# adolliou/euispice_coreg

Measured on AMD Instinct MI355X. Metric: lag-points/sec (whole node) on 2048² grid, 60×60 CRVAL sweep; argmax-shift match, higher is better.
Workload: dtype f64; 1 GPU; headline: Carrington 'fa' 2048x2048 grid lon(200,300) lat(-20,20), 60x60 CRVAL lags arange(-30,30,1) arcsec, small 2048^2 HRIEUV-like, ref 3072^2 FSI-like, order 2, solar_r 1.004; lag_points=3600, parallelism=single GPU, no collective, resident=True, sweeps_in_flight=2, small_stored_f32=True, use_lds=True

## Files before the change

### euispice_coreg_amd/csrc/coreg_hip.hip

```cpp
#include <hip/hip_runtime.h>

#include <algorithm>
#include <chrono>
#include <cmath>
#include <cstdio>
#include <cstdlib>
#include <cstring>
#include <limits>
#include <condition_variable>
#include <map>
#include <memory>
#include <mutex>
#include <string>
#include <thread>
#include <functional>
#include <type_traits>
#include <utility>
#include <vector>

#include "fit.hpp"
#include "geometry.hpp"
#include "kernels.hpp"
#include <atomic>
#include "ricecomp.hpp"
#include "riceenc.hpp"

using namespace coreg;

#define COREG_VERSION "0.1.0"

#include "lag_plan.hpp"
#include "sweep_plan.hpp"
#include "host_owned.hpp"
#include "host_state.hpp"
#include "host_upload.hpp"
#include "host_plan.hpp"
#include "host_fix_launch.hpp"
#include "sweep_variant.hpp"
#include "host_sweep_launch.hpp"
#include "host_sweep_mi.hpp"
#include "host_fix_lists.hpp"
#include "host_sweep_io.hpp"
#include "host_context.hpp"
#include "pixels_plan.hpp"
#include "host_pixels.hpp"

coreg_handle::~coreg_handle() = default;

extern "C" {

const char* coreg_version(void) { return "coreg_hip " COREG_VERSION " (gfx950)"; }

int coreg_create(coreg_handle** out, int device) {
    if (!out) return COREG_EINVAL;
    *out = nullptr;
    int ndev = 0;
    hipError_t e = hipGetDeviceCount(&ndev);
    if (e != hipSuccess || ndev < 1) return COREG_EHIP;
    if (device < 0) {
        if (hipGetDevice(&device) != hipSuccess) device = 0;
    }
    if (device >= ndev) return COREG_EINVAL;
    coreg_handle* h = new (std::nothrow) coreg_handle();
    if (!h) return COREG_ENOMEM;
    h->device = device;
    if (hipSetDevice(device) != hipSuccess || hipStreamCreateWithFlags(&h->stream.s, hipStreamNonBlocking) != hipSuccess ||
        hipEventCreate(&h->ev_end[0].e) != hipSuccess ||
        hipEventCreate(&h->ev_end[1].e) != hipSuccess || hipEventRecord(h->ev_end[0], h->stream) != hipSuccess ||
        hipEventRecord(h->ev_end[1], h->stream) != hipSuccess ||
        h->pivots.reserve(2 * sizeof(double)) != hipSuccess ||
        hipMemsetAsync(h->pivots.p, 0, 2 * sizeof(double), h->stream) != hipSuccess) {
        coreg_destroy(h);
        return COREG_EHIP;
    }
    std::memset(&h->stats, 0, sizeof(h->stats));
    *out = h;
    return COREG_OK;
}

void coreg_destroy(coreg_handle* h) {
    if (!h) return;
    (void)hipSetDevice(h->device);
    if (h->up_thread.joinable()) {
        {
            std::unique_lock<std::mutex> lk(h->up_m);
            h->up_cv.wait(lk, [&] { return !h->up_busy && !h->up_has; });
            h->up_stop = true;
        }
        h->up_cv.notify_all();
        h->up_thread.join();
    }
    if (h->stream) (void)hipStreamSynchronize(h->stream);
    if (h->up_stream) (void)hipStreamSynchronize(h->up_stream);
    delete h;
}

const char* coreg_last_error(const coreg_handle* h) { return h ? h->err.c_str() : "null handle"; }

int coreg_set_stream(coreg_handle* h, void* hip_stream) {
    if (!h) return COREG_EINVAL;
    RETCHK(bind_device(h));
    RETCHK(collect_stats(h));
    HIPCHK(hipStreamSynchronize(h->stream));
    HIPCHK(h->stream.borrow((hipStream_t)hip_stream));
    return COREG_OK;
}

int coreg_synchronize(coreg_handle* h) {
    if (!h) return COREG_EINVAL;
    RETCHK(bind_device(h));
    HIPCHK(hipStreamSynchronize(h->stream));
    return COREG_OK;
}

int coreg_set_option(coreg_handle* h, const char* name, int64_t value) {
    if (!h || !name) return COREG_EINVAL;
    const std::string n(name);
    if (n == "use_lds") {
        h->opt_use_lds = value ? 1 : 0;
    } else if (n == "clean_path") {
        h->opt_clean_path = value ? 1 : 0;
    } else if (n == "tap_nan_filter") {
        if (value < 0 || value > 2) return fail(h, COREG_EINVAL, "tap_nan_filter must be 0, 1 or 2");
        h->opt_tap_nan_filter = value;
    } else if (n == "overlap_upload") {
        h->opt_overlap_upload = value ? 1 : 0;
    } else if (n == "async_upload") {
        h->opt_async_upload = value ? 1 : 0;
    } else if (n == "refine") {
        h->opt_refine = value ? 1 : 0;
    } else if (n == "refine_cond_log10") {
        if (value < -3 || value > 15) return fail(h, COREG_EINVAL, "refine_cond_log10 must be in [-3, 15]");
        h->opt_refine_cond_log10 = value;
    } else if (n == "refine_max") {
        if (value < 0 || value > 16) return fail(h, COREG_EINVAL, "refine_max must be in [0, 16]");
    } else if (n == "tile_w") {
        if (value != 0 && (value < 1 || value > kTilePts || (value & (value - 1)) != 0))
            return fail(h, COREG_EINVAL, "tile_w must be 0 or a power of two <= 1024");
        h->opt_tile_w = value;
    } else if (n == "n_groups") {
        if (value < 0) return fail(h, COREG_EINVAL, "n_groups must be >= 0");
        h->opt_n_groups = value;
    } else if (n == "skew") {
        (void)value;
    } else if (n == "shard_world") {
        if (value < 1 || value > 64) return fail(h, COREG_EINVAL, "shard_world must be in [1, 64]");
        h->opt_shard_world = value;
        if (h->opt_shard_rank >= value) h->opt_shard_rank = 0;
    } else if (n == "combo_begin") {
        if (value < 0) return fail(h, COREG_EINVAL, "combo_begin must be >= 0");
        h->opt_combo_begin = value;
    } else if (n == "combo_end") {
        if (value < 0) return fail(h, COREG_EINVAL, "combo_end must be >= 0");
        h->opt_combo_end = value;
    } else if (n == "shard_rank") {
        if (value < 0 || value >= h->opt_shard_world) return fail(h, COREG_EINVAL, "shard_rank must be in [0, shard_world)");
        h->opt_shard_rank = value;
    } else if (n == "border_fix") {
        h->opt_border_fix = value ? 1 : 0;
    } else if (n == "tap_fix") {
        h->opt_tap_fix = value ? 1 : 0;
    } else if (n == "tap_cap") {
        if (value < 1 || value > (1 << 26)) return fail(h, COREG_EINVAL, "tap_cap must be in [1, 2^26]");
        h->opt_tap_cap = value;
    } else if (n == "pitch") {
        h->opt_pitch = value;
    } else if (n == "taper_frac") {
        if (value < -1 || value > 1000) return fail(h, COREG_EINVAL, "taper_frac must be in [-1, 1000]");
        h->opt_taper_frac = value;
    } else if (n == "taper_min") {
        if (value < 16 || value > 1024) return fail(h, COREG_EINVAL, "taper_min must be in [16, 1024]");
        h->opt_taper_min = value;
    } else if (n == "taper_rounds") {
        if (value < 1) return fail(h, COREG_EINVAL, "taper_rounds must be >= 1");
        h->opt_taper_rounds = value;
    } else if (n == "crop_reference") {
        h->opt_crop_reference = value ? 1 : 0;
    } else if (n == "tile_skip") {
        h->opt_tile_skip = value ? 1 : 0;
    } else if (n == "h_series") {
        h->opt_h_series = value ? 1 : 0;
    } else if (n == "h_incr") {
        h->opt_h_incr = value ? 1 : 0;
    } else if (n == "patch_w") {
        if (value < 0 || value > kBlock) return fail(h, COREG_EINVAL, "patch_w must be in [0, 256]");
        h->opt_patch_w = value;
    } else if (n == "mi_chunks") {
        if (value < 0 || value > kMiMaxChunks) return fail(h, COREG_EINVAL, "mi_chunks must be in [0, 64]");
        h->opt_mi_chunks = value;
    } else if (n == "lds_bytes") {
        if (value < 1024 || value > 159 * 1024) return fail(h, COREG_EINVAL, "lds_bytes must be in [1 KiB, 159 KiB]");
        h->opt_lds_bytes = value;
    } else {
        return fail(h, COREG_EINVAL, "unknown option: " + n);
    }
    return COREG_OK;
}

}

#include "abi_images.hpp"
#include "abi_sweeps.hpp"
#include "abi_host.hpp"
#include "abi_context.hpp"
#include "abi_pixels.hpp"


#include "multi.hpp"
```

### euispice_coreg_amd/csrc/host_state.hpp

```cpp
#pragma once
namespace {

enum SrcKind {
    SRC_HOST = 0,
    SRC_PINNED = 1,
    SRC_DEVICE = 2,
    SRC_TILED = 3,
};

struct PixFmt {
    int bitpix = 0;
    bool f32 = false;
    double bscale = 1.0, bzero = 0.0;
    bool raw() const { return bitpix != 0; }
    bool scaled() const { return bscale != 1.0 || bzero != 0.0; }
    size_t elem() const { return raw() ? (size_t)(bitpix < 0 ? -bitpix : bitpix) / 8 : (f32 ? 4 : 8); }
    bool swap_only() const { return bitpix == -32 && !scaled(); }
    static PixFmt native(bool is_f32) {
        PixFmt f;
        f.f32 = is_f32;
        return f;
    }
};

constexpr int kMaxDevices = 64;
std::mutex g_attr_mutex;

struct EventPair {
    Event a, b;
    bool b_is_next_sweep = false;
    size_t next_sweep_index = 0;
};

}

struct KeptTapLists {
    DevBuf all;
};
struct TapFix {
    TapFixArgs args = {};
    int segs = 0;
    int mode = 0;
    long long count = 0;
};
struct FixLaunch {
    std::vector<BorderFixArgs> border;
    std::vector<ParityFixArgs> parity;
    TapFix tap;
    std::shared_ptr<KeptTapLists> kept;
    bool small_f32 = true;
    bool empty() const { return border.empty() && parity.empty() && tap.segs == 0; }
};

struct ContextState;
struct PixelsState;

struct coreg_handle {
    int device = 0;
    Stream stream;
    std::string err;

    std::unique_ptr<ContextState> ctx;
    std::unique_ptr<PixelsState> pix;
    ~coreg_handle();

    DevBuf small;
    int sW = 0, sH = 0;
    bool small_f32 = false;
    DevBuf ref;
    int gW = 0, gH = 0;
    int ref_dtype = -1;
    DevBuf pivots, red_sum, red_cnt;
    DevBuf t_sin_lon, t_cos_lon, t_cos_lat, t_sin_lat, t_lon_deg, t_dx;
    coreg_diffrot rot_ref = {}, rot_small = {};
    bool has_rot_ref = false, has_rot_small = false;
    CarrTables tabs;
    std::vector<double> tabs_key;
    bool tabs_uploaded = false;
    PinBuf pin_img[2];
    Event ev_img[2];
    int pin_img_next = 0;
    DevBuf pts, tile_count, tile_list, tile_cum, group_first, tile_info, tile_bbox;
    DevBuf visit_rec;
    DevBuf rf_fix_slab;
    DevBuf counters;
    DevBuf lane_params, out_index, partials, out_dev, tmp_img;
    DevBuf counts;
    long long counts_n = -1;
    DevBuf up_f64, up_flag;
    DevBuf up_raw;
    DevBuf rice_blob, rice_rand, dec_img;
    PrologueArgs pending_prologue = {};
    DevBuf bbox_buf;
    Stream aux_stream;
    Stream up_stream;
    Event ev_small, ev_main;
    bool small_pending = false;
    DevBuf red_sum_up, red_cnt_up;
    int64_t opt_overlap_upload = 1;
    int64_t opt_tap_nan_filter = 2;
    int64_t opt_async_upload = 0;
    std::thread up_thread;
    std::mutex up_m;
    std::condition_variable up_cv;
    std::function<hipError_t()> up_job;
    bool up_has = false, up_stop = false, up_busy = false;
    hipError_t up_rc = hipSuccess;
    PinBuf pin_small[2];
    Event ev_pin_small[2];
    int pin_small_next = 0;
    WcslibCaches wcslib;
    DevBuf border_flags, fix_partial;
    DevBuf border_dev;
    PinBuf pin_border;
    int64_t opt_border_fix = 1;
    int64_t opt_tap_fix = 1, opt_tap_cap = 1 << 24;
    DevBuf tap_count, tap_segq, tap_list, tap_skip, tap_seg_slot, tap_seg_begin, tap_pixel, tap_xw, tap_yw;
    long long tap_last[3] = {0, 0, 0};
    int last_variant[7] = {-1, 0, 0, 0, 0, 0, 0};
    int64_t opt_shard_world = 1, opt_shard_rank = 0;
    int64_t opt_combo_begin = 0, opt_combo_end = 0;
    DevBuf sums;
    long long sums_slots = 0;
    struct PendingFinalize {
        long long slot_off, n_slots, lag_begin;
        int residus;
        RefineArgs refine;
        std::function<int(coreg_handle*)> replay_precompute;
        FixLaunch fixes;
    };
    std::function<int(coreg_handle*)> last_precompute;
    PlanMemo plan_memo;
    DevBuf rf_flags, rf_pivots, rf_list, rf_head, rf_partial;
    std::vector<PendingFinalize> pending_fin;
    DevBuf fin_outidx;
    long long pending_n_out = 0;
    std::vector<double> mi_edges_small, mi_edges_large;
    DevBuf mi_hist;
    size_t mi_lds[6] = {0, 0, 0, 0, 0, 0};
    int64_t opt_mi_chunks = 0;

    int64_t opt_crop_reference = 1;
    int64_t opt_taper_min = 128, opt_taper_frac = -1, opt_taper_rounds = 6;
    int64_t opt_use_lds = 1, opt_clean_path = 1, opt_refine = 1, opt_refine_cond_log10 = 5, opt_tile_w = 0, opt_n_groups = 0, opt_lds_bytes = (159 * 1024 * kPointGroups) / 4, opt_patch_w = 0, opt_h_series = 1, opt_h_incr = 1, opt_tile_skip = 1, opt_pitch = -1;

    coreg_stats stats;
    bool stats_pending = false;
    PinBuf pin_info;
    std::vector<EventPair> ev_sweep, ev_pre;
    size_t ev_sweep_used = 0, ev_pre_used = 0;
    hipEvent_t ev_t1 = nullptr;
    Event ev_end[2];
    PinBuf pin_plan[2];
    int plan_slot = 0;
    bool plan_open = false;
};
```

### euispice_coreg_amd/csrc/host_sweep_launch.hpp

```cpp
#pragma once
namespace {
using sweep_variant::SweepVariant;
static_assert(sweep_variant::kTranslate == MODE_TRANSLATE && sweep_variant::kHomography == MODE_HOMOGRAPHY &&
                  sweep_variant::kHomographySeries == MODE_HOMOGRAPHY_SERIES && sweep_variant::kCar == MODE_CAR &&
                  sweep_variant::kOrderRt == ORDER_RT, "sweep_variant.hpp restates the kernels' constants");

struct SweepLaunchSpec {
    int mode = MODE_TRANSLATE;
    int order = 2;
    int method = COREG_METHOD_CORRELATION;
    size_t slot_off = 0;
    int n_batches = 0, n_tiles = 0;
    long long lag_begin = 0;
    double* out_dev = nullptr;
    const LaunchU* car_inv = nullptr;
    const BorderFix* fix = nullptr;
    int pitch_sel = 0;
    long long n_slots() const { return (long long)n_batches * kBlock; }
    bool residus() const { return method != COREG_METHOD_CORRELATION; }
    int residus_kind() const { return method == COREG_METHOD_RESIDUS_MASKED ? 2 : (residus() ? 1 : 0); }
    const double* params_dev(const coreg_handle* h) const {
        return h->lane_params.as<double>() + (mode == MODE_TRANSLATE ? 2 : 9) * slot_off;
    }
    const long long* outidx_dev(const coreg_handle* h) const { return h->out_index.as<long long>() + slot_off; }
};

struct SweepKernel {
    void (*fn)(const SweepArgs);
    size_t attr_bytes[kMaxDevices];
};
template <size_t... I>
SweepKernel* sweep_kernel_table(std::index_sequence<I...>) {
    constexpr const SweepVariant* v = sweep_variant::kSweepVariants.v;
    static SweepKernel table[] = {
        {k_sweep<v[I].mode, v[I].order, std::conditional_t<v[I].f32, float, double>, v[I].round, v[I].resid, v[I].pitch>, {0}}...};
    return table;
}

int raise_dynamic_lds(coreg_handle* h, SweepKernel* k, size_t lds_bytes) {
    std::lock_guard<std::mutex> lock(g_attr_mutex);
    size_t& ab = k->attr_bytes[h->device % kMaxDevices];
    if (lds_bytes > 48 * 1024 && lds_bytes > ab) {
        HIPCHK(hipFuncSetAttribute((const void*)k->fn, hipFuncAttributeMaxDynamicSharedMemorySize, (int)lds_bytes));
        ab = lds_bytes;
    }
    return COREG_OK;
}

int launch_k_sweep(coreg_handle* h, const SweepLaunchSpec& L, const SweepArgs& a, dim3 grid, size_t lds_bytes) {
    const SweepVariant v = sweep_variant::pick_sweep_variant(L.mode, L.order, h->small_f32, L.residus(), L.pitch_sel);
    const int at = sweep_variant::sweep_variant_index(v);
    if (at < 0) return fail(h, COREG_EINVAL, "launch_sweep: no k_sweep instantiation for this mode / order / pitch");
    SweepKernel* k = sweep_kernel_table(std::make_index_sequence<sweep_variant::kNumSweepVariants>()) + at;
    EventPair* ev = next_event(h, h->ev_sweep, h->ev_sweep_used);
    if (!ev) return fail(h, COREG_EHIP, "hipEventCreate failed");
    RETCHK(raise_dynamic_lds(h, k, lds_bytes));
    HIPCHK(hipEventRecord(ev->a, h->stream));
    hipLaunchKernelGGL(k->fn, grid, dim3(kSweepThreads), lds_bytes, h->stream, a);
    HIPCHK(hipEventRecord(ev->b, h->stream));
    HIPCHK(hipGetLastError());
    const int rec[7] = {at, v.mode, v.order, v.f32 ? 1 : 0, v.round ? 1 : 0, v.resid ? 1 : 0, v.pitch};
    std::copy(rec, rec + 7, h->last_variant);
    return COREG_OK;
}

SweepArgs sweep_args(const coreg_handle* h, const SweepLaunchSpec& L, int n_groups, int group_lo, size_t lds_bytes) {
    SweepArgs a;
    a.img = h->small.p;
    a.W = h->sW;
    a.H = h->sH;
    a.pts = h->pts.as<Pt>();
    a.tile_count = h->tile_count.as<int>();
    a.tile_list = h->tile_list.as<int>();
    a.tile_cum = h->tile_cum.as<int>();
    a.group_first = h->group_first.as<int>();
    a.tile_info = h->tile_info.as<long long>();
    a.tile_bbox = h->tile_bbox.as<double>();
    a.visit_rec = h->visit_rec.as<VisitRec>();
    a.lane_params = L.params_dev(h);
    a.n_slots = L.n_slots();
    a.n_batches = L.n_batches;
    a.n_groups = n_groups;
    a.group_lo = group_lo;
    a.partials = h->partials.as<double>();
    a.pivots = h->pivots.as<double>();
    a.use_lds = h->opt_use_lds ? 1 : 0;
    a.clean_path = h->opt_clean_path ? 1 : 0;
    a.lds_elems = (int)(lds_bytes / sizeof(double));
    a.car_inv = L.car_inv ? *L.car_inv : LaunchU{};
    a.car_inv.order_rt = L.order;
    a.car_inv.h_incr = (int)h->opt_h_incr;
    return a;
}

template <typename Args>
void fill_fix_common(Args& x, const coreg_handle* h, const SweepLaunchSpec& L) {
    x.img = h->small.p;
    x.W = h->sW;
    x.H = h->sH;
    x.ref = h->ref.p;
    x.ref_f32 = h->ref_dtype == COREG_F32 ? 1 : 0;
    x.gw = h->gW;
    x.order = L.order;
    x.round_f32 = L.mode == MODE_TRANSLATE ? 0 : 1;
    x.residus = L.residus() ? 1 : 0;
    x.pivots = h->pivots.as<double>();
    x.hom = L.params_dev(h);
    x.n_slots = L.n_slots();
}

int build_fix_launch(coreg_handle* h, const SweepLaunchSpec& L, FixLaunch* fl) {
    fl->small_f32 = h->small_f32;
    if (!L.fix || !L.fix->any()) return COREG_OK;
    static const std::vector<BorderItems::Item> no_items;
    for (const BorderItems::Item& it : L.fix->border ? L.fix->border->items : no_items) {
        if (it.flags_off >= 0) {
            ParityFixArgs p = {};
            fill_fix_common(p, h, L);
            p.flags = h->border_flags.as<unsigned char>() + it.flags_off;
            p.gh = h->gH;
            p.slot = it.slot;
            p.n_partial = 256;
            if (h->fix_partial.reserve((size_t)p.n_partial * kNumSums * sizeof(double)) != hipSuccess)
                return fail(h, COREG_EHIP, "hipMalloc failed (parity fix)");
            p.partial = h->fix_partial.as<double>();
            fl->parity.push_back(p);
        }
        if (it.n == 0) continue;
        BorderFixArgs b = {};
        fill_fix_common(b, h, L);
        b.slot = it.slot;
        b.dropped = h->border_dev.as<int>() + it.first;
        b.n_dropped = it.n;
        fl->border.push_back(b);
    }
    if (L.fix->tap.segs > 0) {
        fl->tap = L.fix->tap;
        fill_fix_common(fl->tap.args, h, L);
    }
    return COREG_OK;
}

int keep_tap_lists(coreg_handle* h, FixLaunch* fixes) {
    auto kept = std::make_shared<KeptTapLists>();
    const size_t nseg = (size_t)fixes->tap.segs, cnt = (size_t)fixes->tap.count;
    TapFixArgs& t = fixes->tap.args;
    const void* src[5] = {t.xw, t.yw, t.pixel, t.seg_begin, t.seg_slot};
    const size_t bytes[5] = {cnt * sizeof(double), cnt * sizeof(double), cnt * sizeof(unsigned), (nseg + 1) * sizeof(int),
                             nseg * sizeof(int)};
    size_t off[6] = {0};
    for (int k = 0; k < 5; ++k) off[k + 1] = off[k] + ((bytes[k] + 7) & ~(size_t)7);
    HIPCHK(kept->all.reserve(off[5]));
    char* all = kept->all.as<char>();
    for (int k = 0; k < 5; ++k)
        if (bytes[k]) HIPCHK(hipMemcpyAsync(all + off[k], src[k], bytes[k], hipMemcpyDeviceToDevice, h->stream));
    t.xw = (const double*)(all + off[0]);
    t.yw = (const double*)(all + off[1]);
    t.pixel = (const unsigned*)(all + off[2]);
    t.seg_begin = (const int*)(all + off[3]);
    t.seg_slot = (const int*)(all + off[4]);
    fixes->kept = kept;
    return COREG_OK;
}

int queue_pending_finalize(coreg_handle* h, const SweepLaunchSpec& L, const RefineArgs& refine, bool refinable,
                           const FixLaunch& fl) {
    coreg_handle::PendingFinalize pf;
    pf.slot_off = (long long)L.slot_off;
    pf.n_slots = L.n_slots();
    pf.lag_begin = L.lag_begin;
    pf.residus = L.residus_kind();
    pf.refine = refine;
    pf.refine.enabled = refinable ? 1 : 0;
    pf.replay_precompute = h->last_precompute;
    pf.fixes = fl;
    if (L.mode == MODE_CAR && fl.tap.segs > 0) RETCHK(keep_tap_lists(h, &pf.fixes));
    h->pending_fin.push_back(pf);
    return COREG_OK;
}

int launch_sweep(coreg_handle* h, const SweepLaunchSpec& L) {
    const long long n_slots = L.n_slots();
    const int n_groups = pick_groups(h, L.n_batches, L.n_tiles);
    const bool sharded = h->opt_shard_world > 1;
    const int g_per = sharded ? n_groups / (int)h->opt_shard_world : n_groups;
    const int g_lo = sharded ? g_per * (int)h->opt_shard_rank : 0;
    const bool fixing = L.fix && L.fix->any() && (!sharded || h->opt_shard_rank == 0);
    HIPCHK(h->partials.reserve((size_t)(g_per + (fixing ? 1 : 0)) * kNumSums * n_slots * sizeof(double)));
    double* fix_slab = fixing ? h->partials.as<double>() + (size_t)g_per * kNumSums * n_slots : nullptr;
    const size_t lds_min = (size_t)(kPointGroups - 1) * kNumSums * kBlock * sizeof(double);
    const size_t lds_bytes = std::max(lds_min, h->opt_use_lds ? (size_t)h->opt_lds_bytes : 0);

    const SweepArgs a = sweep_args(h, L, n_groups, g_lo, lds_bytes);
    RETCHK(join_small(h));
    trace("launch_sweep: launching k_sweep");
    RETCHK(launch_k_sweep(h, L, a, dim3((unsigned)((long long)g_per * L.n_batches)), lds_bytes));
    h->stats.n_sweep_launches++;
    h->stats.used_lds = a.use_lds;

    FixLaunch fl;
    RETCHK(build_fix_launch(h, L, &fl));
    if (fixing) {
        HIPCHK(hipMemsetAsync(fix_slab, 0, (size_t)kNumSums * n_slots * sizeof(double), h->stream));
        RETCHK(launch_fix_kernels(h, fl, fix_slab, nullptr, nullptr));
    }

    const bool refinable = h->opt_refine && !L.residus();
    FinalizeArgs f = {};
    RETCHK(fill_refine(h, &f.refine, L.mode, L.order, a.lane_params, a.car_inv, n_slots));
    f.refine.enabled = (refinable && !sharded) ? 1 : 0;
    if (fixing && f.refine.enabled) {
        HIPCHK(h->rf_fix_slab.reserve((size_t)kNumSums * n_slots * sizeof(double)));
        f.refine.fix_slab = h->rf_fix_slab.as<double>();
    }
    f.fix_slab = fix_slab;
    f.refine_count = h->counters.as<long long>();
    f.partials = h->partials.as<double>();
    f.n_groups = g_per + (fixing ? 1 : 0);
    f.part_stride = n_slots;
    if (sharded) {
        f.sums_out = h->sums.as<double>();
        f.sums_stride = h->sums_slots;
        f.sums_off = (long long)L.slot_off;
    }
    f.n_slots = n_slots;
    f.out_index = L.outidx_dev(h);
    f.lag_begin = L.lag_begin;
    f.out = L.out_dev;
    f.counts = h->counts.as<double>();
    f.residus = L.residus_kind();
    f.n_required = (long long)h->gW * h->gH;
    launch_finalize(h, f);
    HIPCHK(hipGetLastError());

    if (sharded) return queue_pending_finalize(h, L, f.refine, refinable, fl);
    if (!f.refine.enabled) return COREG_OK;
    hipLaunchKernelGGL(k_refine_list, dim3(1), dim3(kListThreads), 0, h->stream, f.refine, n_slots, h->counters.as<long long>());
    return refine_with_fixes(h, f.refine, fl, n_slots, f.out_index, L.lag_begin, L.out_dev);
}

}
```

### euispice_coreg_amd/csrc/kernels_sweep.hpp

```cpp
#pragma once
namespace coreg {
struct SweepArgs {
    const void* img;
    int W, H;
    const Pt* pts;
    const int* tile_count;
    const int* tile_list;
    const int* tile_cum;
    const int* group_first;
    long long* tile_info;
    const double* tile_bbox;
    const VisitRec* visit_rec;
    const double* lane_params;
    long long n_slots;
    int n_batches;
    int n_groups;
    int group_lo;
    double* partials;
    const double* pivots;
    int use_lds;
    int clean_path;
    int lds_elems;
    LaunchU car_inv;
};

struct Acc {
    int n;
    double a, b, aa, bb, ab;
};

template <int N>
struct Taps;
template <>
struct Taps<3> {
    double t[9];
    __device__ __forceinline__ void issue(unsigned a0, unsigned a1, unsigned a2) {
        asm volatile(
            "ds_read_b64 %0, %9\n\tds_read_b64 %1, %9 offset:8\n\tds_read_b64 %2, %9 offset:16\n\t"
            "ds_read_b64 %3, %10\n\tds_read_b64 %4, %10 offset:8\n\tds_read_b64 %5, %10 offset:16\n\t"
            "ds_read_b64 %6, %11\n\tds_read_b64 %7, %11 offset:8\n\tds_read_b64 %8, %11 offset:16"
            : "=&v"(t[0]), "=&v"(t[1]), "=&v"(t[2]), "=&v"(t[3]), "=&v"(t[4]), "=&v"(t[5]), "=&v"(t[6]), "=&v"(t[7]),
              "=&v"(t[8])
            : "v"(a0), "v"(a1), "v"(a2));
    }
    __device__ __forceinline__ void wait_after(double& w0, double& w1, double& w2, double& w3, double& w4, double& w5) {
        asm volatile("s_waitcnt lgkmcnt(0)"
                     : "+v"(t[0]), "+v"(t[1]), "+v"(t[2]), "+v"(t[3]), "+v"(t[4]), "+v"(t[5]), "+v"(t[6]), "+v"(t[7]),
                       "+v"(t[8]), "+v"(w0), "+v"(w1), "+v"(w2), "+v"(w3), "+v"(w4), "+v"(w5));
    }
    __device__ __forceinline__ void issue_before(unsigned a0, unsigned a1, unsigned a2, double& fx, double& fy) {
        asm volatile(
            "ds_read_b64 %0, %11\n\tds_read_b64 %1, %11 offset:8\n\tds_read_b64 %2, %11 offset:16\n\t"
            "ds_read_b64 %3, %12\n\tds_read_b64 %4, %12 offset:8\n\tds_read_b64 %5, %12 offset:16\n\t"
            "ds_read_b64 %6, %13\n\tds_read_b64 %7, %13 offset:8\n\tds_read_b64 %8, %13 offset:16"
            : "=&v"(t[0]), "=&v"(t[1]), "=&v"(t[2]), "=&v"(t[3]), "=&v"(t[4]), "=&v"(t[5]), "=&v"(t[6]), "=&v"(t[7]),
              "=&v"(t[8]), "+v"(fx), "+v"(fy)
            : "v"(a0), "v"(a1), "v"(a2));
    }
    __device__ __forceinline__ void wait() {
        asm volatile("s_waitcnt lgkmcnt(0)"
                     : "+v"(t[0]), "+v"(t[1]), "+v"(t[2]), "+v"(t[3]), "+v"(t[4]), "+v"(t[5]), "+v"(t[6]), "+v"(t[7]),
                       "+v"(t[8]));
    }
    template <int P>
    __device__ __forceinline__ void issue_before_imm(unsigned a0, double& fx, double& fy) {
        static_assert(P > 0 && (2 * P + 2) * 8 < 65536, "LDS immediate offsets are 16 bits");
        asm volatile(
            "ds_read_b64 %0, %11\n\tds_read_b64 %1, %11 offset:8\n\tds_read_b64 %2, %11 offset:16\n\t"
            "ds_read_b64 %3, %11 offset:%12\n\tds_read_b64 %4, %11 offset:%13\n\tds_read_b64 %5, %11 offset:%14\n\t"
            "ds_read_b64 %6, %11 offset:%15\n\tds_read_b64 %7, %11 offset:%16\n\tds_read_b64 %8, %11 offset:%17"
            : "=&v"(t[0]), "=&v"(t[1]), "=&v"(t[2]), "=&v"(t[3]), "=&v"(t[4]), "=&v"(t[5]), "=&v"(t[6]), "=&v"(t[7]),
              "=&v"(t[8]), "+v"(fx), "+v"(fy)
            : "v"(a0), "n"(P * 8), "n"(P * 8 + 8), "n"(P * 8 + 16), "n"(2 * P * 8), "n"(2 * P * 8 + 8),
              "n"(2 * P * 8 + 16));
    }
};
template <>
struct Taps<2> {
    double t[4];
    __device__ __forceinline__ void issue(unsigned a0, unsigned a1, unsigned) {
        asm volatile(
            "ds_read_b64 %0, %4\n\tds_read_b64 %1, %4 offset:8\n\t"
            "ds_read_b64 %2, %5\n\tds_read_b64 %3, %5 offset:8"
            : "=&v"(t[0]), "=&v"(t[1]), "=&v"(t[2]), "=&v"(t[3])
            : "v"(a0), "v"(a1));
    }
    __device__ __forceinline__ void issue_before(unsigned a0, unsigned a1, unsigned a2, double&, double&) {
        issue(a0, a1, a2);
    }
    __device__ __forceinline__ void wait_after(double&, double&, double&, double&, double&, double&) { wait(); }
    __device__ __forceinline__ void wait() {
        asm volatile("s_waitcnt lgkmcnt(0)" : "+v"(t[0]), "+v"(t[1]), "+v"(t[2]), "+v"(t[3]));
    }
};

template <>
struct Taps<4> {
    double t[16];
    __device__ __forceinline__ void issue_before(unsigned a0, unsigned a1, unsigned a2, unsigned a3, double& fx,
                                                 double& fy) {
        asm volatile(
            "ds_read_b64 %0, %18\n\tds_read_b64 %1, %18 offset:8\n\tds_read_b64 %2, %18 offset:16\n\t"
            "ds_read_b64 %3, %18 offset:24\n\t"
            "ds_read_b64 %4, %19\n\tds_read_b64 %5, %19 offset:8\n\tds_read_b64 %6, %19 offset:16\n\t"
            "ds_read_b64 %7, %19 offset:24\n\t"
            "ds_read_b64 %8, %20\n\tds_read_b64 %9, %20 offset:8\n\tds_read_b64 %10, %20 offset:16\n\t"
            "ds_read_b64 %11, %20 offset:24\n\t"
            "ds_read_b64 %12, %21\n\tds_read_b64 %13, %21 offset:8\n\tds_read_b64 %14, %21 offset:16\n\t"
            "ds_read_b64 %15, %21 offset:24"
            : "=&v"(t[0]), "=&v"(t[1]), "=&v"(t[2]), "=&v"(t[3]), "=&v"(t[4]), "=&v"(t[5]), "=&v"(t[6]), "=&v"(t[7]),
              "=&v"(t[8]), "=&v"(t[9]), "=&v"(t[10]), "=&v"(t[11]), "=&v"(t[12]), "=&v"(t[13]), "=&v"(t[14]),
              "=&v"(t[15]), "+v"(fx), "+v"(fy)
            : "v"(a0), "v"(a1), "v"(a2), "v"(a3));
    }
    template <int P>
    __device__ __forceinline__ void issue_before_imm(unsigned a0, double& fx, double& fy) {
        static_assert(P > 0 && (3 * P + 3) * 8 < 65536, "LDS immediate offsets are 16 bits");
        asm volatile(
            "ds_read_b64 %0, %18\n\tds_read_b64 %1, %18 offset:8\n\tds_read_b64 %2, %18 offset:16\n\t"
            "ds_read_b64 %3, %18 offset:24\n\t"
            "ds_read_b64 %4, %18 offset:%19\n\tds_read_b64 %5, %18 offset:%20\n\tds_read_b64 %6, %18 offset:%21\n\t"
            "ds_read_b64 %7, %18 offset:%22\n\t"
            "ds_read_b64 %8, %18 offset:%23\n\tds_read_b64 %9, %18 offset:%24\n\tds_read_b64 %10, %18 offset:%25\n\t"
            "ds_read_b64 %11, %18 offset:%26\n\t"
            "ds_read_b64 %12, %18 offset:%27\n\tds_read_b64 %13, %18 offset:%28\n\tds_read_b64 %14, %18 offset:%29\n\t"
            "ds_read_b64 %15, %18 offset:%30"
            : "=&v"(t[0]), "=&v"(t[1]), "=&v"(t[2]), "=&v"(t[3]), "=&v"(t[4]), "=&v"(t[5]), "=&v"(t[6]), "=&v"(t[7]),
              "=&v"(t[8]), "=&v"(t[9]), "=&v"(t[10]), "=&v"(t[11]), "=&v"(t[12]), "=&v"(t[13]), "=&v"(t[14]),
              "=&v"(t[15]), "+v"(fx), "+v"(fy)
            : "v"(a0), "n"(P * 8), "n"(P * 8 + 8), "n"(P * 8 + 16), "n"(P * 8 + 24), "n"(2 * P * 8), "n"(2 * P * 8 + 8),
              "n"(2 * P * 8 + 16), "n"(2 * P * 8 + 24), "n"(3 * P * 8), "n"(3 * P * 8 + 8), "n"(3 * P * 8 + 16),
              "n"(3 * P * 8 + 24));
    }
    __device__ __forceinline__ void wait_after(double* wx, double* wy) {
        asm volatile("s_waitcnt lgkmcnt(0)"
                     : "+v"(t[0]), "+v"(t[1]), "+v"(t[2]), "+v"(t[3]), "+v"(t[4]), "+v"(t[5]), "+v"(t[6]), "+v"(t[7]),
                       "+v"(t[8]), "+v"(t[9]), "+v"(t[10]), "+v"(t[11]), "+v"(t[12]), "+v"(t[13]), "+v"(t[14]),
                       "+v"(t[15]), "+v"(wx[0]), "+v"(wx[1]), "+v"(wx[2]), "+v"(wx[3]), "+v"(wy[0]), "+v"(wy[1]),
                       "+v"(wy[2]), "+v"(wy[3]));
    }
};

template <int PITCH, bool FOLDED = false>
__device__ __forceinline__ double gather_o3(unsigned win, int pitch, double cx, double cy, double offx, double offy) {
    int c0, r0;
    double fx, fy;
    if constexpr (FOLDED) {
        c0 = (int)cx;
        r0 = (int)cy;
        fx = __builtin_amdgcn_fract(cx);
        fy = __builtin_amdgcn_fract(cy);
    } else {
        const double flx = floor(cx), fly = floor(cy);
        c0 = (int)flx + (int)offx;
        r0 = (int)fly + (int)offy;
        fx = cx - flx;
        fy = cy - fly;
    }
    const unsigned a0 = win + 8u * (unsigned)(__mul24(r0, PITCH > 0 ? PITCH : pitch) + c0);
    Taps<4> tp;
    if constexpr (PITCH > 0) {
        tp.template issue_before_imm<PITCH>(a0, fx, fy);
    } else {
        const unsigned a1 = a0 + 8u * (unsigned)pitch;
        const unsigned a2 = a1 + 8u * (unsigned)pitch;
        const unsigned a3 = a2 + 8u * (unsigned)pitch;
        tp.issue_before(a0, a1, a2, a3, fx, fy);
    }
    double wx[4], wy[4];
    spline_weights6_o3(fx, wx);
    spline_weights6_o3(fy, wy);
// ... 328 lines not shown
        const unsigned lo = (unsigned)__builtin_amdgcn_readlane(w, 3 + 2 * k);
        const unsigned hi = (unsigned)__builtin_amdgcn_readlane(w, 4 + 2 * k);
        b[k] = __builtin_bit_cast(double, ((unsigned long long)hi << 32) | (unsigned long long)lo);
    }
    v.bx0 = b[0];
    v.bx1 = b[1];
    v.by0 = b[2];
    v.by1 = b[3];
}

template <int MODE, int ORDER, typename TS, bool LDS, bool ROUND, bool RESID, bool INTERIOR = false, int PITCH = 0,
          bool CLEAN = false>
__device__ __forceinline__ void tile_points(Acc& acc, unsigned win, const TS* __restrict__ img, int pitch,
                                            int ox, int oy, int W, int H, double px0, double py0, double pxw,
                                            double pyw, const H9& hm, const LaunchU& cu, const Pt* __restrict__ pts, int p_begin, int p_end,
                                            double pivot_b, int pg) {
    const double wmax = (double)(W - 1), hmax = (double)(H - 1);
    const int n_full = p_end / kChunk;
#if defined(__HIP_DEVICE_COMPILE__) && COREG_PT_SCALAR == 2
    constexpr bool kIncr = INTERIOR && LDS && ORDER == 2 && !RESID &&
                           (MODE == MODE_HOMOGRAPHY || MODE == MODE_HOMOGRAPHY_SERIES);
    if constexpr (kIncr) {
        if (cu.h_incr) {
            H9 hv = hm;
            hv.h[0] = fma(pxw, hm.h[6], hm.h[0]);
            hv.h[1] = fma(pxw, hm.h[7], hm.h[1]);
            hv.h[2] = MODE == MODE_HOMOGRAPHY_SERIES ? hm.h[2] + pxw : fma(pxw, hm.h[8], hm.h[2]);
            hv.h[3] = fma(pyw, hm.h[6], hm.h[3]);
            hv.h[4] = fma(pyw, hm.h[7], hm.h[4]);
            hv.h[5] = MODE == MODE_HOMOGRAPHY_SERIES ? hm.h[5] + pyw : fma(pyw, hm.h[8], hm.h[5]);
            int c = p_begin / kChunk + pg;
            if (c < n_full) {
                double& anchor = hv.h[7];
                SPt cur = spt_load(pts + c * kChunk, anchor);
                spt_wait(cur);
                for (; c < n_full; c += kPointGroups) {
                    const Pt* __restrict__ q = pts + c * kChunk;
                    const bool run = cur[7] != 0u;
                    double xn = 0.0, yn = 0.0, ww = 0.0;
#pragma unroll
                    for (int k = 0; k < kChunk; ++k) {
                        SPt nxt = spt_load(k + 1 < kChunk ? q + k + 1 : q + kPointGroups * kChunk, anchor);
                        const double x = spt_f64(cur, 0), y = spt_f64(cur, 1);
                        if (k == 0 || !run) {
                            xn = fma(hv.h[0], x, fma(hv.h[1], y, hv.h[2]));
                            yn = fma(hv.h[3], x, fma(hv.h[4], y, hv.h[5]));
                            ww = MODE == MODE_HOMOGRAPHY_SERIES ? fma(hv.h[6], x, hv.h[7] * y)
                                                                : fma(hv.h[6], x, fma(hv.h[7], y, hv.h[8]));
                        } else {
                            xn += hv.h[0];
                            yn += hv.h[3];
                            ww += hv.h[6];
                        }
                        double ux, uy;
                        if (MODE == MODE_HOMOGRAPHY_SERIES) {
                            const double qq = fma(ww, ww, -ww);
                            ux = fma(xn, qq, xn);
                            uy = fma(yn, qq, yn);
                        } else {
                            double r = __builtin_amdgcn_rcp(ww);
                            r = fma(r, fma(-ww, r, 1.0), r);
                            ux = xn * r;
                            uy = yn * r;
                        }
                        point_lag<MODE, ORDER, TS, LDS, ROUND, RESID, INTERIOR, PITCH, CLEAN, true>(
                            acc, win, img, pitch, ox, oy, W, H, wmax, hmax, px0, py0, pxw, pyw, hv, cu, ux, uy,
                            spt_f64(cur, 2), spt_f64(cur, 3), pivot_b);
                        if constexpr (CLEAN) {
                            if (k == 1) acc.a += spt_f64(cur, 3);
                            if (k == 2) acc.aa += spt_f64(cur, 3);
                            if (k == kChunk - 1) acc.n += kChunk;
                        }
                        spt_wait(nxt);
                        cur = nxt;
                    }
                }
            }
            if (pg == n_full % kPointGroups) {
                for (int p = n_full * kChunk; p < p_end; ++p) {
                    Pt pt;
                    load_pt_uniform(pts + p, pt);
                    point_lag<MODE, ORDER, TS, LDS, ROUND, RESID, INTERIOR, PITCH>(acc, win, img, pitch, ox, oy, W, H, wmax,
                                                                                   hmax, px0, py0, pxw, pyw, hm, cu, pt.b0,
                                                                                   pt.b1, pt.a, pt.pad, pivot_b);
                }
            }
            return;
        }
    }
    {
        int c = p_begin / kChunk + pg;
        if (c < n_full) {
            H9 hml = hm;
            double& anchor = MODE == MODE_TRANSLATE ? (INTERIOR && LDS ? pxw : px0) : hml.h[MODE == MODE_CAR ? 0 : 7];
            SPt cur = spt_load(pts + c * kChunk, anchor);
            spt_wait(cur);
            for (; c < n_full; c += kPointGroups) {
                const Pt* __restrict__ q = pts + c * kChunk;
#pragma unroll
                for (int k = 0; k < kChunk; ++k) {
                    SPt nxt = spt_load(k + 1 < kChunk ? q + k + 1 : q + kPointGroups * kChunk, anchor);
                    point_lag<MODE, ORDER, TS, LDS, ROUND, RESID, INTERIOR, PITCH, CLEAN>(
                        acc, win, img, pitch, ox, oy, W, H, wmax, hmax, px0, py0, pxw, pyw, hml, cu, spt_f64(cur, 0),
                        spt_f64(cur, 1), spt_f64(cur, 2), spt_f64(cur, 3), pivot_b);
                    if constexpr (CLEAN) {
                        if (k == 1) acc.a += spt_f64(cur, 3);
                        if (k == 2) acc.aa += spt_f64(cur, 3);
                        if (k == kChunk - 1) acc.n += kChunk;
                    }
                    spt_wait(nxt);
                    cur = nxt;
                }
            }
        }
    }
#else
    for (int c = p_begin / kChunk + pg; c < n_full; c += kPointGroups) {
        const Pt* __restrict__ q = pts + c * kChunk;
        Pt pt[kChunk];
#pragma unroll
        for (int k = 0; k < kChunk; ++k) load_pt_uniform(q + k, pt[k]);
#pragma unroll
        for (int k = 0; k < kChunk; ++k)
            point_lag<MODE, ORDER, TS, LDS, ROUND, RESID, INTERIOR, PITCH, CLEAN>(acc, win, img, pitch, ox, oy, W, H, wmax,
                                                                                  hmax, px0, py0, pxw, pyw, hm, cu, pt[k].b0,
                                                                                  pt[k].b1, pt[k].a, pt[k].pad, pivot_b);
        if constexpr (CLEAN) {
            acc.n += kChunk;
            acc.a += pt[1].pad;
            acc.aa += pt[2].pad;
        }
    }
#endif
    if (pg == n_full % kPointGroups) {
        for (int p = n_full * kChunk; p < p_end; ++p) {
            Pt pt;
            load_pt_uniform(pts + p, pt);
            point_lag<MODE, ORDER, TS, LDS, ROUND, RESID, INTERIOR, PITCH>(acc, win, img, pitch, ox, oy, W, H, wmax, hmax,
                                                                           px0, py0, pxw, pyw, hm, cu, pt.b0, pt.b1, pt.a,
                                                                           pt.pad, pivot_b);
        }
    }
}

template <int MODE, int ORDER, typename TS, bool ROUND, bool RESID, int PITCH = 0>
__global__ void __launch_bounds__(kSweepThreads) k_sweep(const SweepArgs a) {
    extern __shared__ __align__(16) unsigned char lds_raw[];
    double* lds = (double*)lds_raw;
    constexpr int kWaves = kSweepThreads / 64;
    constexpr int kLagWaves = kBlock / 64;
    __shared__ double wred2[2][kLagWaves][4];
    __shared__ int wdirty[2][kWaves];
    constexpr bool kCleanPath = MODE != MODE_CAR && !RESID && ORDER != ORDER_RT && !(ROUND && sizeof(TS) == 8);
    int visit = 0;
    int n_vis = 0, n_vis_lds = 0, n_vis_int = 0, n_vis_clean = 0;

    const int b = blockIdx.x;
    const int slot8 = b & 7;
    const int q = b >> 3;
    const int batch = q % a.n_batches;
    const int group = a.group_lo + (q / a.n_batches) * 8 + slot8;

    const int lane = threadIdx.x & 63, wave = threadIdx.x >> 6;
    const int pg = __builtin_amdgcn_readfirstlane(wave % kPointGroups);
    const int lw = __builtin_amdgcn_readfirstlane(wave / kPointGroups);
    const int ls = 64 * lw + lane;
    const long long slot = (long long)batch * kBlock + ls;

    double px0 = 0.0, py0 = 0.0;
    H9 hm;
#pragma unroll
    for (int k = 0; k < 9; ++k) hm.h[k] = 0.0;
    if (MODE == MODE_TRANSLATE) {
        px0 = a.lane_params[slot];
        py0 = a.lane_params[a.n_slots + slot];
    } else {
#pragma unroll
        for (int k = 0; k < 9; ++k) hm.h[k] = a.lane_params[(long long)k * a.n_slots + slot];
    }

    const bool pad_lane = MODE == MODE_TRANSLATE ? (px0 != px0) : (hm.h[8] != hm.h[8]);

    Acc acc = {0, 0.0, 0.0, 0.0, 0.0, 0.0};

    const TS* __restrict__ img = (const TS*)a.img;
    const int W = a.W, H = a.H;
    const double inf = __builtin_inf();
    const int u_lo = a.group_first[1024 + group];
    const int u_hi = a.group_first[1024 + group + 1];
    const double pivot_b = a.pivots[1];
#if defined(__HIP_DEVICE_COMPILE__)
    const unsigned win = (unsigned)(uintptr_t)(__attribute__((address_space(3))) unsigned char*)lds_raw;
#else
    const unsigned win = 0;
#endif

    constexpr bool kLagBox = MODE == MODE_TRANSLATE && COREG_VISIT_LAGBOX;
    double lx0 = 0.0, lx1 = 0.0, ly0 = 0.0, ly1 = 0.0;
    if constexpr (kLagBox) {
        lx0 = lx1 = px0;
        ly0 = ly1 = py0;
        for (int o = 32; o > 0; o >>= 1) {
            lx0 = fmin(lx0, __shfl_xor(lx0, o));
            lx1 = fmax(lx1, __shfl_xor(lx1, o));
            ly0 = fmin(ly0, __shfl_xor(ly0, o));
            ly1 = fmax(ly1, __shfl_xor(ly1, o));
        }
        if (lane == 0 && pg == 0) {
            wred2[0][lw][0] = lx0;
            wred2[0][lw][1] = lx1;
            wred2[0][lw][2] = ly0;
            wred2[0][lw][3] = ly1;
        }
        __syncthreads();
        lx0 = fmin(fmin(wred2[0][0][0], wred2[0][1][0]), fmin(wred2[0][2][0], wred2[0][3][0]));
        lx1 = fmax(fmax(wred2[0][0][1], wred2[0][1][1]), fmax(wred2[0][2][1], wred2[0][3][1]));
        ly0 = fmin(fmin(wred2[0][0][2], wred2[0][1][2]), fmin(wred2[0][2][2], wred2[0][3][2]));
        ly1 = fmax(fmax(wred2[0][0][3], wred2[0][1][3]), fmax(wred2[0][2][3], wred2[0][3][3]));
    }

    int tl = a.group_first[group];
    unsigned park = 0;
    {
        Visit first;
        load_visit_uniform(a.visit_rec + tl, first);
        park = park_visit(first, park);
    }
    for (; u_lo < u_hi; ++tl) {
        Visit cur;
        unpark_visit(park, cur);
        const int ubase = cur.ubase;
        if (ubase >= u_hi) break;
        Visit nxt;
        load_visit_uniform(a.visit_rec + tl + 1, nxt);
        const int tile = cur.tile;
        const int cnt = cur.cnt;
        const int p_begin = max(u_lo - ubase, 0) * kUnitPts;
        const int p_end = min((u_hi - ubase) * kUnitPts, cnt);
        if (p_begin >= p_end) {
            park = park_visit(nxt, park);
            continue;
        }
        const double bx0 = cur.bx0, bx1 = cur.bx1, by0 = cur.by0, by1 = cur.by1;

        double mnx, mxx, mny, mxy;
        if constexpr (kLagBox) {
            mnx = bx0 + lx0;
            mxx = bx1 + lx1;
            mny = by0 + ly0;
            mxy = by1 + ly1;
        } else if (MODE == MODE_TRANSLATE) {
            mnx = bx0 + px0;
            mxx = bx1 + px0;
            mny = by0 + py0;
            mxy = by1 + py0;
        } else {
            mnx = inf; mxx = -inf; mny = inf; mxy = -inf;
#pragma unroll
            for (int c = 0; c < 4; ++c) {
                double cx, cy;
                apply_map<MODE>(hm, a.car_inv, (c & 1) ? bx1 : bx0, (c & 2) ? by1 : by0, cx, cy);
                mnx = fmin(mnx, cx);
                mxx = fmax(mxx, cx);
                mny = fmin(mny, cy);
                mxy = fmax(mxy, cy);
            }
            if (MODE == MODE_CAR) {
                const double margin = car_tile_margin(a.car_inv.box_c, fmax(fabs(by0), fabs(by1)) + a.car_inv.pole_sep);
                mnx -= margin;
                mxx += margin;
                mny -= margin;
                mxy += margin;
            }
        }
        int* wdirt = wdirty[visit & 1];
        if constexpr (!kLagBox) {
            for (int o = 32; o > 0; o >>= 1) {
                mnx = fmin(mnx, __shfl_xor(mnx, o));
                mxx = fmax(mxx, __shfl_xor(mxx, o));
                mny = fmin(mny, __shfl_xor(mny, o));
                mxy = fmax(mxy, __shfl_xor(mxy, o));
            }
            double(*wred)[4] = wred2[visit & 1];
            if (lane == 0 && pg == 0) {
                wred[lw][0] = mnx;
                wred[lw][1] = mxx;
                wred[lw][2] = mny;
                wred[lw][3] = mxy;
            }
            __syncthreads();
            mnx = fmin(fmin(wred[0][0], wred[1][0]), fmin(wred[2][0], wred[3][0]));
            mxx = fmax(fmax(wred[0][1], wred[1][1]), fmax(wred[2][1], wred[3][1]));
            mny = fmin(fmin(wred[0][2], wred[1][2]), fmin(wred[2][2], wred[3][2]));
            mxy = fmax(fmax(wred[0][3], wred[1][3]), fmax(wred[2][3], wred[3][3]));
        }
        ++visit;
        if (!(mxx >= 0.0) || !(mnx <= (double)(W - 1)) || !(mxy >= 0.0) || !(mny <= (double)(H - 1))) {
            park = park_visit(nxt, park);
            continue;
        }
        if constexpr (kLagBox) __syncthreads();
        constexpr double kClear = 1e-9;
        const bool interior = (mnx >= kClear) & (mxx <= (double)(W - 1) - kClear) & (mny >= kClear) &
                              (mxy <= (double)(H - 1) - kClear);
        constexpr bool kWide = ORDER == ORDER_RT || ORDER > 2;
        const int ord = ORDER == ORDER_RT ? a.car_inv.order_rt : ORDER;
        const int ap_lo = kWide ? ord / 2 + 1 : 1;
        const int ap_hi = kWide ? ord - ord / 2 + 1 : 2;
        const int ox = max((int)floor(fmax(mnx, 0.0)) - ap_lo, kWide ? -ap_lo : -1);
        const int oy = max((int)floor(fmax(mny, 0.0)) - ap_lo, kWide ? -ap_lo : -1);
        const int ex = min((int)floor(fmin(mxx, (double)(W - 1))) + ap_hi, kWide ? W - 1 + ap_hi : W);
        const int ey = min((int)floor(fmin(mxy, (double)(H - 1))) + ap_hi, kWide ? H - 1 + ap_hi : H);
        const int ww = ex - ox + 1, wh = ey - oy + 1;
        int pitch = PITCH > 0 ? PITCH : (ww | 1);
        if (PITCH == 0) {
            const int r = pitch & 31;
            const int up = r < 5 ? 5 - r : ((r > 11 && r < 21) ? 21 - r : (r > 27 ? 37 - r : 0));
            if ((long long)(pitch + up) * wh <= (long long)a.lds_elems) pitch += up;
        }
        const long long need = (long long)pitch * wh;
        const bool in_lds = a.use_lds && (need <= (long long)a.lds_elems) && (PITCH == 0 || ww <= PITCH);

        const Pt* __restrict__ pts = a.pts + (size_t)tile * kTilePts;

        bool swept = false;
        ++n_vis;
        {
          if (in_lds) {
            swept = true;
            ++n_vis_lds;
#ifndef COREG_STAGE_ROWS
#define COREG_STAGE_ROWS 8
#endif
#ifndef COREG_STAGE_COLS
#define COREG_STAGE_COLS 1
#endif
            constexpr int kStage = COREG_STAGE_ROWS, kCols = COREG_STAGE_COLS;
            const double scale = ORDER == 2 ? 0.25 : 1.0;
            constexpr bool kFmaStage = ORDER == 2 && !ROUND && COREG_VISIT_FMA;
            const double npivot4 = -0.25 * pivot_b;
            const int wave_u = __builtin_amdgcn_readfirstlane(wave);
            double poison = 0.0;
            for (int r0 = wave_u; r0 < wh; r0 += kWaves * kStage) {
                for (int c0 = 0; c0 < ww; c0 += 64 * kCols) {
                    int gx[kCols];
#pragma unroll
                    for (int j = 0; j < kCols; ++j) {
                        const int c = c0 + 64 * j + lane;
                        gx[j] = kWide ? mirror_far(ox + min(c, ww - 1), W) : mirror_idx(ox + min(c, ww - 1), W);
                    }
                    TS v[kStage][kCols];
#pragma unroll
                    for (int k = 0; k < kStage; ++k) {
                        const int r = min(r0 + k * kWaves, wh - 1);
                        const int gy = kWide ? mirror_far(oy + r, H) : mirror_idx(oy + r, H);
                        const TS* __restrict__ row = img + (size_t)gy * W;
#pragma unroll
                        for (int j = 0; j < kCols; ++j) v[k][j] = row[gx[j]];
                    }
#pragma unroll
                    for (int j = 0; j < kCols; ++j) {
                        const int c = c0 + 64 * j + lane;
                        if (c < ww) {
#pragma unroll
                            for (int k = 0; k < kStage; ++k) {
                                const int r = r0 + k * kWaves;
                                if (r < wh) {
                                    const double e = (kFmaStage ? fma((double)v[k][j], 0.25, npivot4)
                                                                : (ROUND ? (double)v[k][j] : (double)v[k][j] - pivot_b) * scale);
                                    lds[r * pitch + c] = e;
                                    if (kCleanPath) poison = fma(e, 0.0, poison);
                                }
                            }
                        }
                    }
                }
            }
            park = park_visit(nxt, park);
            if (kCleanPath && interior) {
                const int dirty = __ballot(poison != poison) != 0ull;
                if (lane == 0) wdirt[wave] = dirty;
            }
            __syncthreads();
            bool done = false;
            if constexpr (ORDER != ORDER_RT) {
                if (interior) {
                    done = true;
                    bool clean = false;
                    if constexpr (kCleanPath) clean = a.clean_path && __ballot(wdirt[lane % kWaves] != 0) == 0ull;
                    ++n_vis_int;
                    n_vis_clean += clean ? 1 : 0;
                    if (!pad_lane) {
                        const double offx = (ORDER == 2 ? 0.5 : 0.0) - (double)(ORDER / 2 + ox);
                        const double offy = (ORDER == 2 ? 0.5 : 0.0) - (double)(ORDER / 2 + oy);
                        const double pxw = MODE == MODE_TRANSLATE ? px0 + offx : offx;
                        const double pyw = MODE == MODE_TRANSLATE ? py0 + offy : offy;
                        if (kCleanPath && clean) {
                            tile_points<MODE, ORDER, TS, true, ROUND, RESID, true, PITCH, kCleanPath>(
                                acc, win, img, pitch, ox, oy, W, H, px0, py0, pxw, pyw, hm, a.car_inv, pts, p_begin, p_end,
                                pivot_b, pg);
                        } else {
                            tile_points<MODE, ORDER, TS, true, ROUND, RESID, true, PITCH>(acc, win, img, pitch, ox, oy, W, H,
                                                                                          px0, py0, pxw, pyw, hm, a.car_inv,
                                                                                          pts, p_begin, p_end, pivot_b, pg);
                        }
                    }
                }
            }
            if (!done) {
                const double offx = ORDER == 2 ? 0.5 - (double)(1 + ox) : (ORDER == 3 ? -(double)(1 + ox) : 0.0);
                const double offy = ORDER == 2 ? 0.5 - (double)(1 + oy) : (ORDER == 3 ? -(double)(1 + oy) : 0.0);
                tile_points<MODE, ORDER, TS, true, ROUND, RESID, false, PITCH>(acc, win, img, pitch, ox, oy, W, H, px0, py0,
                                                                               offx, offy, hm, a.car_inv, pts, p_begin,
                                                                               p_end, pivot_b, pg);
            }
          }
        }
        if (!swept) {
            park = park_visit(nxt, park);
            tile_points<MODE, ORDER, TS, false, ROUND, RESID>(acc, win, img, 0, 0, 0, W, H, px0, py0, 0.0, 0.0, hm, a.car_inv, pts,
                                                              p_begin, p_end, pivot_b, pg);
        }
    }

    if (threadIdx.x == 0) {
        atomicAdd((unsigned long long*)a.tile_info + 3, (unsigned long long)n_vis);
        atomicAdd((unsigned long long*)a.tile_info + 4, (unsigned long long)n_vis_lds);
        atomicAdd((unsigned long long*)a.tile_info + 5, (unsigned long long)n_vis_int);
        atomicAdd((unsigned long long*)a.tile_info + 6, (unsigned long long)n_vis_clean);
    }
    __syncthreads();
    if (pg > 0) {
        double* st = lds + ((size_t)(pg - 1) * kNumSums) * kBlock + ls;
        st[0] = (double)acc.n;
        st[kBlock] = acc.a;
        st[2 * kBlock] = acc.b;
        st[3 * kBlock] = acc.aa;
        st[4 * kBlock] = acc.bb;
        st[5 * kBlock] = acc.ab;
    }
    __syncthreads();
    if (pg == 0) {
        double sn = (double)acc.n, sa = acc.a, sb = acc.b, saa = acc.aa, sbb = acc.bb, sab = acc.ab;
        for (int g = 0; g < kPointGroups - 1; ++g) {
            const double* st = lds + ((size_t)g * kNumSums) * kBlock + ls;
            sn += st[0];
            sa += st[kBlock];
            sb += st[2 * kBlock];
            saa += st[3 * kBlock];
            sbb += st[4 * kBlock];
            sab += st[5 * kBlock];
        }
        double* out = a.partials + (size_t)(group - a.group_lo) * kNumSums * a.n_slots + slot;
        out[0] = sn;
        out[a.n_slots] = sa;
        out[2 * a.n_slots] = sb;
        out[3 * a.n_slots] = saa;
        out[4 * a.n_slots] = sbb;
        out[5 * a.n_slots] = sab;
    }
}

}
```

Measured before the change: 1.237 million lag-points/s.

## Make k_sweep persistent with an atomic work queue sized to device residency

Converts the sweep kernel from one workgroup per (group, batch) item into a persistent kernel. The grid is capped at the number of resident workgroups, computed from the CU count and occupancy and cached per kernel and LDS size. Each workgroup pulls further items from a per-slot8 atomic ticket counter. This aims to cut workgroup launch and scheduling overhead and to balance uneven tile work dynamically. In exchange it adds a memset and atomics per launch, a double-buffered next-item broadcast, and a requirement that groups per launch be a multiple of 8.

```diff
diff --git a/euispice_coreg_amd/csrc/coreg_hip.hip b/euispice_coreg_amd/csrc/coreg_hip.hip
--- a/euispice_coreg_amd/csrc/coreg_hip.hip
+++ b/euispice_coreg_amd/csrc/coreg_hip.hip
@@ -141,6 +141,9 @@
     } else if (n == "n_groups") {
         if (value < 0) return fail(h, COREG_EINVAL, "n_groups must be >= 0");
         h->opt_n_groups = value;
+    } else if (n == "sweep_wgs") {
+        if (value < 0) return fail(h, COREG_EINVAL, "sweep_wgs must be >= 0");
+        h->opt_sweep_wgs = value;
     } else if (n == "skew") {
         (void)value;
     } else if (n == "shard_world") {
diff --git a/euispice_coreg_amd/csrc/host_state.hpp b/euispice_coreg_amd/csrc/host_state.hpp
--- a/euispice_coreg_amd/csrc/host_state.hpp
+++ b/euispice_coreg_amd/csrc/host_state.hpp
@@ -85,6 +85,15 @@
     DevBuf rf_fix_slab;
     DevBuf counters;
     DevBuf lane_params, out_index, partials, out_dev, tmp_img;
+    DevBuf sweep_queue;
+    int n_cus = 0;
+    struct SweepResidency {
+        const void* fn;
+        size_t lds_bytes;
+        int per_cu;
+    };
+    std::vector<SweepResidency> sweep_residency;
+    int64_t opt_sweep_wgs = 0;
     DevBuf counts;
     long long counts_n = -1;
     DevBuf up_f64, up_flag;
diff --git a/euispice_coreg_amd/csrc/host_sweep_launch.hpp b/euispice_coreg_amd/csrc/host_sweep_launch.hpp
--- a/euispice_coreg_amd/csrc/host_sweep_launch.hpp
+++ b/euispice_coreg_amd/csrc/host_sweep_launch.hpp
@@ -47,7 +47,25 @@
     return COREG_OK;
 }
 
-int launch_k_sweep(coreg_handle* h, const SweepLaunchSpec& L, const SweepArgs& a, dim3 grid, size_t lds_bytes) {
+int sweep_grid(coreg_handle* h, const SweepKernel* k, size_t lds_bytes, long long items, unsigned* grid) {
+    long long resident = h->opt_sweep_wgs;
+    if (resident <= 0) {
+        if (h->n_cus <= 0) HIPCHK(hipDeviceGetAttribute(&h->n_cus, hipDeviceAttributeMultiprocessorCount, h->device));
+        int per_cu = 0;
+        for (const coreg_handle::SweepResidency& r : h->sweep_residency)
+            if (r.fn == (const void*)k->fn && r.lds_bytes == lds_bytes) per_cu = r.per_cu;
+        if (per_cu <= 0) {
+            HIPCHK(hipOccupancyMaxActiveBlocksPerMultiprocessor(&per_cu, (const void*)k->fn, kSweepThreads, lds_bytes));
+            if (per_cu <= 0) return fail(h, COREG_EHIP, "launch_sweep: the device holds no k_sweep workgroup of this LDS size");
+            h->sweep_residency.push_back({(const void*)k->fn, lds_bytes, per_cu});
+        }
+        resident = (long long)h->n_cus * per_cu;
+    }
+    *grid = (unsigned)(8 * ((std::min(items, resident) + 7) / 8));
+    return COREG_OK;
+}
+
+int launch_k_sweep(coreg_handle* h, const SweepLaunchSpec& L, SweepArgs a, int n_groups8, size_t lds_bytes) {
     const SweepVariant v = sweep_variant::pick_sweep_variant(L.mode, L.order, h->small_f32, L.residus(), L.pitch_sel);
     const int at = sweep_variant::sweep_variant_index(v);
     if (at < 0) return fail(h, COREG_EINVAL, "launch_sweep: no k_sweep instantiation for this mode / order / pitch");
@@ -55,8 +73,14 @@
     EventPair* ev = next_event(h, h->ev_sweep, h->ev_sweep_used);
     if (!ev) return fail(h, COREG_EHIP, "hipEventCreate failed");
     RETCHK(raise_dynamic_lds(h, k, lds_bytes));
+    a.items8 = n_groups8 * L.n_batches;
+    unsigned grid = 0;
+    RETCHK(sweep_grid(h, k, lds_bytes, 8LL * a.items8, &grid));
+    HIPCHK(h->sweep_queue.reserve(8 * sizeof(unsigned)));
+    a.queue = h->sweep_queue.as<unsigned>();
+    HIPCHK(hipMemsetAsync(a.queue, 0, 8 * sizeof(unsigned), h->stream));
     HIPCHK(hipEventRecord(ev->a, h->stream));
-    hipLaunchKernelGGL(k->fn, grid, dim3(kSweepThreads), lds_bytes, h->stream, a);
+    hipLaunchKernelGGL(k->fn, dim3(grid), dim3(kSweepThreads), lds_bytes, h->stream, a);
     HIPCHK(hipEventRecord(ev->b, h->stream));
     HIPCHK(hipGetLastError());
     const int rec[7] = {at, v.mode, v.order, v.f32 ? 1 : 0, v.round ? 1 : 0, v.resid ? 1 : 0, v.pitch};
@@ -83,6 +107,8 @@
     a.n_groups = n_groups;
     a.group_lo = group_lo;
     a.partials = h->partials.as<double>();
+    a.queue = nullptr;
+    a.items8 = 0;
     a.pivots = h->pivots.as<double>();
     a.use_lds = h->opt_use_lds ? 1 : 0;
     a.clean_path = h->opt_clean_path ? 1 : 0;
@@ -194,7 +220,8 @@
     const SweepArgs a = sweep_args(h, L, n_groups, g_lo, lds_bytes);
     RETCHK(join_small(h));
     trace("launch_sweep: launching k_sweep");
-    RETCHK(launch_k_sweep(h, L, a, dim3((unsigned)((long long)g_per * L.n_batches)), lds_bytes));
+    if (g_per % 8 != 0) return fail(h, COREG_EINVAL, "launch_sweep: the groups of a launch must be a multiple of 8");
+    RETCHK(launch_k_sweep(h, L, a, g_per / 8, lds_bytes));
     h->stats.n_sweep_launches++;
     h->stats.used_lds = a.use_lds;
 
diff --git a/euispice_coreg_amd/csrc/kernels_sweep.hpp b/euispice_coreg_amd/csrc/kernels_sweep.hpp
--- a/euispice_coreg_amd/csrc/kernels_sweep.hpp
+++ b/euispice_coreg_amd/csrc/kernels_sweep.hpp
@@ -17,6 +17,8 @@
     int n_groups;
     int group_lo;
     double* partials;
+    unsigned* queue;
+    int items8;
     const double* pivots;
     int use_lds;
     int clean_path;
@@ -651,20 +653,33 @@
     __shared__ double wred2[2][kLagWaves][4];
     __shared__ int wdirty[2][kWaves];
     constexpr bool kCleanPath = MODE != MODE_CAR && !RESID && ORDER != ORDER_RT && !(ROUND && sizeof(TS) == 8);
-    int visit = 0;
     int n_vis = 0, n_vis_lds = 0, n_vis_int = 0, n_vis_clean = 0;
 
-    const int b = blockIdx.x;
-    const int slot8 = b & 7;
-    const int q = b >> 3;
-    const int batch = q % a.n_batches;
-    const int group = a.group_lo + (q / a.n_batches) * 8 + slot8;
+    __shared__ int next_q[2];
+    const int slot8 = blockIdx.x & 7;
+    int q = blockIdx.x >> 3;
+    int item_par = 0;
 
     const int lane = threadIdx.x & 63, wave = threadIdx.x >> 6;
     const int pg = __builtin_amdgcn_readfirstlane(wave % kPointGroups);
     const int lw = __builtin_amdgcn_readfirstlane(wave / kPointGroups);
     const int ls = 64 * lw + lane;
+
+    const TS* __restrict__ img = (const TS*)a.img;
+    const int W = a.W, H = a.H;
+    const double inf = __builtin_inf();
+    const double pivot_b = a.pivots[1];
+#if defined(__HIP_DEVICE_COMPILE__)
+    const unsigned win = (unsigned)(uintptr_t)(__attribute__((address_space(3))) unsigned char*)lds_raw;
+#else
+    const unsigned win = 0;
+#endif
+
+    while (q < a.items8) {
+    const int batch = q % a.n_batches;
+    const int group = a.group_lo + (q / a.n_batches) * 8 + slot8;
     const long long slot = (long long)batch * kBlock + ls;
+    int visit = 0;
 
     double px0 = 0.0, py0 = 0.0;
     H9 hm;
@@ -682,17 +697,8 @@
 
     Acc acc = {0, 0.0, 0.0, 0.0, 0.0, 0.0};
 
-    const TS* __restrict__ img = (const TS*)a.img;
-    const int W = a.W, H = a.H;
-    const double inf = __builtin_inf();
     const int u_lo = a.group_first[1024 + group];
     const int u_hi = a.group_first[1024 + group + 1];
-    const double pivot_b = a.pivots[1];
-#if defined(__HIP_DEVICE_COMPILE__)
-    const unsigned win = (unsigned)(uintptr_t)(__attribute__((address_space(3))) unsigned char*)lds_raw;
-#else
-    const unsigned win = 0;
-#endif
 
     constexpr bool kLagBox = MODE == MODE_TRANSLATE && COREG_VISIT_LAGBOX;
     double lx0 = 0.0, lx1 = 0.0, ly0 = 0.0, ly1 = 0.0;
@@ -922,13 +928,10 @@
         }
     }
 
-    if (threadIdx.x == 0) {
-        atomicAdd((unsigned long long*)a.tile_info + 3, (unsigned long long)n_vis);
-        atomicAdd((unsigned long long*)a.tile_info + 4, (unsigned long long)n_vis_lds);
-        atomicAdd((unsigned long long*)a.tile_info + 5, (unsigned long long)n_vis_int);
-        atomicAdd((unsigned long long*)a.tile_info + 6, (unsigned long long)n_vis_clean);
-    }
+    unsigned ticket = 0;
+    if (threadIdx.x == 0) ticket = atomicAdd(a.queue + slot8, 1u);
     __syncthreads();
+    if (threadIdx.x == 0) next_q[item_par] = (int)(gridDim.x >> 3) + (int)ticket;
     if (pg > 0) {
         double* st = lds + ((size_t)(pg - 1) * kNumSums) * kBlock + ls;
         st[0] = (double)acc.n;
@@ -958,6 +961,16 @@
         out[4 * a.n_slots] = sbb;
         out[5 * a.n_slots] = sab;
     }
-}
-
-}
+    q = __builtin_amdgcn_readfirstlane(next_q[item_par]);
+    item_par ^= 1;
+    }
+
+    if (threadIdx.x == 0) {
+        atomicAdd((unsigned long long*)a.tile_info + 3, (unsigned long long)n_vis);
+        atomicAdd((unsigned long long*)a.tile_info + 4, (unsigned long long)n_vis_lds);
+        atomicAdd((unsigned long long*)a.tile_info + 5, (unsigned long long)n_vis_int);
+        atomicAdd((unsigned long long*)a.tile_info + 6, (unsigned long long)n_vis_clean);
+    }
+}
+
+}
```

Measured after the change: 1.267 million lag-points/s, median of 6. 2.5% higher.
